# jjjkkyz/NU-NeRF

Measured on AMD Instinct MI355X. Metric: train rays/sec, higher is better.
Workload: dtype f32

## Files before the change

nu_nerf_amd/csrc/gemm.h:

```cpp
#pragma once
#include "nu_common.h"

#include "nu_nerf.h"

int nu_gemm_nt_launch(const NuGemmNT& g, hipStream_t stream);
int nu_gemm_nt_batch_launch(const NuGemmNT* probs, int n, hipStream_t stream);
int nu_gemm_tn_launch(const NuGemmTN& g, hipStream_t stream);
int nu_reduce_push(NuReduceDesc* descs, int* ndesc, int cap, const float* slab, int S, int N1, int N2, int rs,
                   long long ss, float* out, int ldo, float alpha, int accumulate);

int nu_ctx_take(NuOpCtx* c, long long nbytes, int ndesc_needed, hipStream_t stream, float** out, long long* out_bytes);
void nu_ctx_ev_begin(NuOpCtx* c, hipStream_t stream);
void nu_ctx_ev_end(NuOpCtx* c, hipStream_t stream, double kind, double flops, double bytes);
```

nu_nerf_amd/csrc/gemm_epi.h:

```cpp
#pragma once
#include "gemm.h"
#include <type_traits>

#define TBM 128
#define TBN 128
#define TBK 32
#define NT_LDS 36
#define NT_LDSH 40
#define NT_WPC 3

#define EPI_LDS 68

template <int EPI>
static __device__ inline float nu_epi_apply(float v, float bv, float h, float d, float ca, float& out2) {
    out2 = 0.f;
    if (EPI == NU_EPI_BIAS_NONE) return v + bv;
    if (EPI == NU_EPI_BIAS_RELU) return fmaxf(v + bv, 0.0f);
    if (EPI == NU_EPI_BIAS_SOFTPLUS) return nu_softplus100_fast(v + bv);
    if (EPI == NU_EPI_MUL_DRELU) return h > 0.0f ? v : 0.0f;
    if (EPI == NU_EPI_MUL_DSP) return v * (1.0f - nu_exp_m100(h));
    if (EPI == NU_EPI_Q_SP) {
        const float e = nu_exp_m100(h);
        out2 = v * d * 100.0f * e;
        return v * (1.0f - e);
    }
    if (EPI == NU_EPI_B_SP) return v * (1.0f - nu_exp_m100(h)) + ca;
    if (EPI == NU_EPI_B_RELU) return (h > 0.0f ? v : 0.0f) + ca;
    return v;
}

template <int EPI>
struct NtEpiArgs {
    float* C; float* C2; const float* bias; const float* H; const float* D; const float* Cadd;
    unsigned long long* mask;
    int zero_to, act_cols;
    bool vec_ok;
    bool c16, x16;
    static constexpr bool kMaskW = (EPI == NU_EPI_BIAS_RELU);
    static constexpr bool kMaskR = (EPI == NU_EPI_MUL_DRELU || EPI == NU_EPI_B_RELU);
    static constexpr bool kNeedH = (EPI == NU_EPI_MUL_DRELU || EPI == NU_EPI_MUL_DSP || EPI == NU_EPI_Q_SP ||
                                    EPI == NU_EPI_B_SP || EPI == NU_EPI_B_RELU);
    static constexpr bool kNeedD = (EPI == NU_EPI_Q_SP);
    static constexpr bool kNeedAdd = (EPI == NU_EPI_B_SP || EPI == NU_EPI_B_RELU);
    static constexpr bool kBias = (EPI <= NU_EPI_BIAS_SOFTPLUS);
};

template <int EPI, bool H16 = false>
static __device__ inline NtEpiArgs<EPI> nt_epi_args(const NuGemmNT& g, int z) {
    typedef NtEpiArgs<EPI> E;
    E a;
    a.c16 = H16 && (g.bf16 & NU_GEMM_C16) != 0;
    a.x16 = H16 && (g.bf16 & NU_GEMM_X16) != 0;
    const int ec = a.c16 ? 2 : 4, ex = a.x16 ? 2 : 4;
    auto off = [](const float* p, long long elems, int eb) { return reinterpret_cast<const float*>(reinterpret_cast<const char*>(p) + elems * eb); };
    a.C = const_cast<float*>(off(g.C, (long long)z * g.sC, ec));
    a.C2 = g.C2 ? const_cast<float*>(off(g.C2, (long long)z * g.sC2, ec)) : nullptr;
    a.bias = g.bias ? g.bias + (long long)z * g.sBias : nullptr;
    a.H = g.H ? off(g.H, (long long)z * g.sH, ex) : nullptr;
    a.D = g.D ? off(g.D, (long long)z * g.sD, ex) : nullptr;
    a.Cadd = g.Cadd ? off(g.Cadd, (long long)z * g.sCadd, ex) : nullptr;
    a.zero_to = g.zero_to > g.N ? g.zero_to : g.N;
    a.act_cols = g.act_cols > 0 ? g.act_cols : 0x7fffffff;
    a.mask = (E::kMaskW || E::kMaskR) ? g.mask : nullptr;
    const uintptr_t mc = a.c16 ? 7 : 15, mx = a.x16 ? 7 : 15;
    bool v = (((uintptr_t)a.C & mc) == 0) && ((g.ldc & 3) == 0);
    if (E::kNeedH) v = v && (((uintptr_t)a.H & mx) == 0) && ((g.ldh & 3) == 0);
    if (E::kNeedD) v = v && (((uintptr_t)a.D & mx) == 0) && ((g.ldd & 3) == 0) && (((uintptr_t)a.C2 & mc) == 0) && ((g.ldc2 & 3) == 0);
    if (E::kNeedAdd) v = v && (((uintptr_t)a.Cadd & mx) == 0) && ((g.ldadd & 3) == 0);
    a.vec_ok = v;
    return a;
}

static __device__ __forceinline__ f32x4 nu_bf16x4_to_f32(uint2 r) {
    f32x4 o;
    o[0] = __uint_as_float(r.x << 16); o[1] = __uint_as_float(r.x & 0xffff0000u);
// ... 17 lines not shown
    else base[idx] = v;
}

template <int EPI>
static __device__ inline unsigned long long* nt_mask_words(const NtEpiArgs<EPI>& ea, const NuGemmNT& g, int mt, int nt, int z, int ntn, int wid) {
    const int ct = g.mask_ct0 + z * ntn + nt;
    return (ea.mask && ct < g.mask_nct) ? ea.mask + ((((long long)mt * g.mask_nct + ct) * 4 + wid) * 64) : nullptr;
}

template <int EPI, int NBH, bool H16 = false, int TMN = 2>
static __device__ __forceinline__ void nt_epilogue(const NuGemmNT& g, const NtEpiArgs<EPI>& ea, f32x16 (&acc)[TMN][2], float* scr,
                                                   int m0, int n0, unsigned long long* mwave, unsigned mlo, unsigned mhi,
                                                   int lane, int wid, int tm0 = 0) {
    typedef NtEpiArgs<EPI> E;
    constexpr bool kMaskW = E::kMaskW, kMaskR = E::kMaskR, kNeedH = E::kNeedH, kNeedD = E::kNeedD, kNeedAdd = E::kNeedAdd, kBias = E::kBias;
    float* const C = ea.C; float* const C2 = ea.C2;
    const float* const bias = ea.bias; const float* const H = ea.H; const float* const D = ea.D; const float* const Cadd = ea.Cadd;
    const int zero_to = ea.zero_to, act_cols = ea.act_cols;
    const bool vec_ok = ea.vec_ok;
    const bool c16 = H16 && ea.c16, x16 = H16 && ea.x16;
    const int ec = c16 ? 2 : 4, ex = x16 ? 2 : 4;
    const int li = lane & 31, lh = lane >> 5;
    const int wr = wid >> 1, wc = wid & 1;
    unsigned wlo = 0, whi = 0;
    const int colq = (lane & 15) * 4;
    const int gcol = n0 + wc * 64 + colq;
    float bv[4] = {0.f, 0.f, 0.f, 0.f};
    if (kBias && bias) {
#pragma unroll
        for (int e = 0; e < 4; ++e) bv[e] = (gcol + e < g.N) ? bias[gcol + e] : 0.f;
    }
    const bool full = vec_ok && (gcol + 3 < g.N) && (gcol + 3 < act_cols || gcol >= act_cols);
    const int wcol0 = n0 + wc * 64, wrow0 = m0 + wr * 64;
    const bool slab_full = vec_ok && (wrow0 + 64 <= g.M) && (wcol0 + 64 <= g.N) && (wcol0 + 64 <= act_cols || wcol0 >= act_cols);
    const bool slab_plain = kNeedH && wcol0 >= act_cols;
    const int uwid = __builtin_amdgcn_readfirstlane(wid);
    const long long urow0 = m0 + (uwid >> 1) * 64, ucol0 = n0 + (uwid & 1) * 64;
    const unsigned lrow = lane >> 4;
    char* const Cu = reinterpret_cast<char*>(C) + (urow0 * g.ldc + ucol0) * ec;
    char* const C2u = kNeedD ? reinterpret_cast<char*>(C2) + (urow0 * g.ldc2 + ucol0) * ec : nullptr;
    const char* const Hu = kNeedH ? reinterpret_cast<const char*>(H) + (urow0 * g.ldh + ucol0) * ex : nullptr;
    const char* const Du = kNeedD ? reinterpret_cast<const char*>(D) + (urow0 * g.ldd + ucol0) * ex : nullptr;
    const char* const Au = kNeedAdd ? reinterpret_cast<const char*>(Cadd) + (urow0 * g.ldadd + ucol0) * ex : nullptr;
    const unsigned oC = (lrow * (unsigned)g.ldc + (unsigned)colq) * (unsigned)ec, oC2 = (lrow * (unsigned)g.ldc2 + (unsigned)colq) * (unsigned)ec;
    const unsigned oH = (lrow * (unsigned)g.ldh + (unsigned)colq) * (unsigned)ex, oD = (lrow * (unsigned)g.ldd + (unsigned)colq) * (unsigned)ex;
    const unsigned oA = (lrow * (unsigned)g.ldadd + (unsigned)colq) * (unsigned)ex;
#pragma unroll
    for (int tt = 0; tt < TMN; ++tt) {
        const int tm = tm0 + tt;
#pragma unroll
        for (int tn = 0; tn < 2; ++tn)
#pragma unroll
            for (int r = 0; r < 16; ++r)
                scr[((r & 3) + 8 * (r >> 2) + 4 * lh) * EPI_LDS + tn * 32 + li] = acc[tt][tn][r];
        if (slab_full) {
            auto fast = [&](auto ub_c, auto pl_c, auto c16_c, auto x16_c) {
                constexpr bool UB = decltype(ub_c)::value, PL = decltype(pl_c)::value;
                constexpr bool c16 = decltype(c16_c)::value, x16 = decltype(x16_c)::value;
                constexpr int ec = c16 ? 2 : 4, ex = x16 ? 2 : 4;
                constexpr int NB = kNeedH ? NBH : 4;
#pragma unroll
                for (int hb = 0; hb < 8 / NB; ++hb) {
                    f32x4 v4[NB], h4[NB], d4[NB], c4v[NB];
#pragma unroll
                    for (int ii = 0; ii < NB; ++ii) {
                        const int i = hb * NB + ii;
                        const long long roff = (long long)(tm * 32 + i * 4);
                        v4[ii] = *reinterpret_cast<const f32x4*>(&scr[(i * 4 + (lane >> 4)) * EPI_LDS + colq]);
                        if (kNeedH && !PL && !UB) h4[ii] = nt_ld4<H16>(Hu + roff * g.ldh * ex + oH, x16);
                        if (kNeedD && !PL) d4[ii] = nt_ld4<H16>(Du + roff * g.ldd * ex + oD, x16);
                        if (kNeedAdd && !PL) c4v[ii] = nt_ld4<H16>(Au + roff * g.ldadd * ex + oA, x16);
                    }
#pragma unroll
                    for (int ii = 0; ii < NB; ++ii) {
                        const int i = hb * NB + ii;
                        const long long roff = (long long)(tm * 32 + i * 4);
                        f32x4 o4, o24;
#pragma unroll
                        for (int e = 0; e < 4; ++e) {
                            float o2 = 0.f;
                            const float v = g.alpha * v4[ii][e];
                            if constexpr (PL) {
                                o4[e] = v;
                            } else if constexpr (kMaskR && UB) {
                                const int src = (tm * 8 + i) * 4 + e;
                                const unsigned long long w = ((unsigned long long)(unsigned)__builtin_amdgcn_readlane(mhi, src) << 32) |
                                                             (unsigned)__builtin_amdgcn_readlane(mlo, src);
                                float sel;
                                asm("s_nop 1\n\tv_cndmask_b32_e64 %0, 0, %1, %2" : "=v"(sel) : "v"(v), "s"(w));
                                o4[e] = kNeedAdd ? sel + c4v[ii][e] : sel;
                            } else {
                                o4[e] = nu_epi_apply<EPI>(v, bv[e], kNeedH ? h4[ii][e] : 0.f, kNeedD ? d4[ii][e] : 0.f,
                                                          kNeedAdd ? c4v[ii][e] : 0.f, o2);
                            }
                            o24[e] = o2;
                        }
                        nt_st4<H16>(Cu + roff * g.ldc * ec + oC, o4, c16);
                        if (kNeedD) nt_st4<H16>(C2u + roff * g.ldc2 * ec + oC2, o24, c16);
                        if constexpr (kMaskW && UB) {
#pragma unroll
                            for (int e = 0; e < 4; ++e) {
                                const unsigned long long bits = __ballot(o4[e] > 0.f);
                                const bool mine = lane == (tm * 8 + i) * 4 + e;
                                wlo = mine ? (unsigned)bits : wlo;
                                whi = mine ? (unsigned)(bits >> 32) : whi;
                            }
                        }
                    }
// ... 26 lines not shown
                if (row < g.M) {
                if (full) {
                    f32x4 h4 = {0.f, 0.f, 0.f, 0.f}, d4 = h4, c4v = h4, o4, o24;
                    const bool plain = gcol >= act_cols;
                    if (kMaskR && mwave) {
                        if (!plain) {
#pragma unroll
                            for (int e = 0; e < 4; ++e) {
                                const int src = (tm * 8 + i) * 4 + e;
                                const unsigned lo = __builtin_amdgcn_readlane(mlo, src), hi = __builtin_amdgcn_readlane(mhi, src);
                                h4[e] = (((lane < 32 ? lo : hi) >> (lane & 31)) & 1u) ? 1.0f : 0.0f;
                            }
                        }
                    } else if (kNeedH && !plain) h4 = nt_ld4<H16>(reinterpret_cast<const char*>(H) + ((long long)row * g.ldh + gcol) * ex, x16);
                    if (kNeedD && !plain) d4 = nt_ld4<H16>(reinterpret_cast<const char*>(D) + ((long long)row * g.ldd + gcol) * ex, x16);
                    if (kNeedAdd && !plain) c4v = nt_ld4<H16>(reinterpret_cast<const char*>(Cadd) + ((long long)row * g.ldadd + gcol) * ex, x16);
#pragma unroll
                    for (int e = 0; e < 4; ++e) {
                        float o2;
                        const float v = g.alpha * v4[e];
                        o4[e] = (kNeedH && plain) ? v : nu_epi_apply<EPI>(v, bv[e], h4[e], d4[e], c4v[e], o2);
                        o24[e] = (kNeedH && plain) ? 0.f : o2;
                    }
                    nt_st4<H16>(reinterpret_cast<char*>(C) + ((long long)row * g.ldc + gcol) * ec, o4, c16);
                    if (kNeedD) nt_st4<H16>(reinterpret_cast<char*>(C2) + ((long long)row * g.ldc2 + gcol) * ec, o24, c16);
                    if (kMaskW) {
#pragma unroll
                        for (int e = 0; e < 4; ++e) pos[e] = o4[e] > 0.f;
                    }
                } else {
#pragma unroll
                    for (int e = 0; e < 4; ++e) {
                        const int col = gcol + e;
                        if (col >= zero_to) continue;
                        float out = 0.f, out2 = 0.f;
                        if (col < g.N) {
                            const float v = g.alpha * v4[e];
                            if (kNeedH && col >= act_cols) {
                                out = v;
                            } else {
                                const float h = kNeedH ? nt_ld1<H16>(H, (long long)row * g.ldh + col, x16) : 0.f;
                                const float d = kNeedD ? nt_ld1<H16>(D, (long long)row * g.ldd + col, x16) : 0.f;
                                const float ca = kNeedAdd ? nt_ld1<H16>(Cadd, (long long)row * g.ldadd + col, x16) : 0.f;
                                out = nu_epi_apply<EPI>(v, bv[e], h, d, ca, out2);
                            }
                        }
                        nt_st1<H16>(C, (long long)row * g.ldc + col, out, c16);
                        if (kNeedD) nt_st1<H16>(C2, (long long)row * g.ldc2 + col, out2, c16);
                    }
                }
                }
                if (kMaskW && mwave) {
#pragma unroll
                    for (int e = 0; e < 4; ++e) {
                        const unsigned long long bits = __ballot(pos[e]);
                        const bool mine = lane == (tm * 8 + i) * 4 + e;
                        wlo = mine ? (unsigned)bits : wlo;
                        whi = mine ? (unsigned)(bits >> 32) : whi;
// ... 9 lines not shown
```

nu_nerf_amd/csrc/gemm_nt.hip:

```cpp
#include "gemm_epi.h"

template <int EPI, int PREC>
__global__ __launch_bounds__(256, PREC == 2 ? 2 : NT_WPC) void gemm_nt_kernel(NuGemmNT g) {
    static_assert(PREC == 1 || PREC == 2, "gemm_nt_kernel covers the bf16 modes only");
    constexpr bool SPLIT = PREC == 2;
    constexpr int kPlane = TBM * NT_LDSH;
    __shared__ __attribute__((aligned(16))) float smem[SPLIT ? 1 : 2][SPLIT ? 3 * kPlane : TBM * NT_LDS];
    __bf16* const hA = reinterpret_cast<__bf16*>(&smem[0][0]);
    __bf16* const hB = hA + (SPLIT ? 3 : 1) * kPlane;

    const int tid = threadIdx.x;
    const int lane = tid & 63;
    const int wid = tid >> 6;
    const int wr = wid >> 1, wc = wid & 1;
    const int z = blockIdx.z;
    const int ntn = (g.N + TBN - 1) / TBN;
    const int mtiles = (g.M + TBM - 1) / TBM;
    const int nslots = ((mtiles + 7) / 8) * 8 * ntn;

    const float* __restrict__ A = g.A + (long long)z * g.sA;
    const float* __restrict__ B = g.B + (long long)z * g.sB;
    const int c4 = tid & 7;
    const int r0 = tid >> 3;
    const int nk = g.K / TBK;
// ... 318 lines not shown
#undef NT2_PIN
        nt_epilogue<EPI, 4, false, TMN>(g, ea, acc, &smem[(cur ^ 1) * NT2_STAGE] + wid * (32 * EPI_LDS), m0, n0, mwave, mlo, mhi, lane, slab, tm0);
        int mtn = 0, ntnx = 0;
        const int jn = next_valid(j + gridDim.x, pi, mtn, ntnx);
        if (jn >= nslots) break;
        __syncthreads();
        j = jn; mt = mtn; nt = ntnx;
    }
}

template <int EPI, int TMN>
__global__ __launch_bounds__(256, 2) void gemm_nt2_kernel(NuGemmNT g) {
    __shared__ __attribute__((aligned(16))) float smem[2 * NT2_STAGE];
    nt2_run<EPI, TMN, false>(&g, nullptr, 1, smem);
}
template <int EPI, int TMN>
__global__ __launch_bounds__(256, 2) void gemm_nt2b_kernel(NuGemmNTBatch b) {
    __shared__ __attribute__((aligned(16))) float smem[2 * NT2_STAGE];
    nt2_run<EPI, TMN, true>(b.p, b.slot0, b.n, smem);
}

int nu_gemm_nt16_launch(const NuGemmNT& g, int groups, long long nslots, hipStream_t stream);
int nu_gemm_nt6_launch(const NuGemmNT& g, int groups, hipStream_t stream);

static int nt_check(const NuGemmNT& g) {
    if (g.N <= 0 || g.K <= 0 || (g.K % TBK) != 0 || g.lda < g.K || g.ldb < g.K) return NU_ERR_ARG;
    if ((g.lda & 3) || (g.ldb & 3)) return NU_ERR_ARG;
    if (((uintptr_t)g.A & 15) || ((uintptr_t)g.B & 15)) return NU_ERR_ARG;
    const int ntn = nu_cdiv(g.N, TBN);
    const long long nslots = (long long)nu_rup(nu_cdiv(g.M, 64), 8) * ntn;
    if (nslots > 0x7fffffffLL) return NU_ERR_ARG;
    const int groups = g.groups > 0 ? g.groups : 1;
    if (g.mask && (g.epi == NU_EPI_BIAS_RELU || g.epi == NU_EPI_MUL_DRELU || g.epi == NU_EPI_B_RELU)) {
        if ((g.N & 3) || (g.ldc & 3) || ((uintptr_t)g.C & 15) || g.mask_nct <= 0 || g.mask_ct0 < 0) return NU_ERR_ARG;
        if (g.epi == NU_EPI_B_RELU && ((g.ldadd & 3) || ((uintptr_t)g.Cadd & 15))) return NU_ERR_ARG;
        if (g.epi == NU_EPI_BIAS_RELU && ((long long)g.mask_ct0 + (long long)groups * ntn > g.mask_nct || (g.N & 63))) return NU_ERR_ARG;
        if (g.act_cols > 0 && (g.act_cols & 63)) return NU_ERR_ARG;
    }
    const int prec = g.bf16 & 3;
    if (prec == 3) return NU_ERR_ARG;
    if ((g.bf16 & ~3) && !(prec == 1 && (g.bf16 & NU_GEMM_B16)) && !(prec == 2 && (g.bf16 & ~3) == NU_GEMM_PRESPLIT_ALWAYS && g.B6))
        return NU_ERR_ARG;
    return NU_OK;
}

static bool nt_small_tiles(long long t128, long long t64) {
    auto round_eff = [&](long long tiles) { return (double)tiles / (double)(nu_cdivl(tiles, 512) * 512); };
    return t128 < 512 || 0.95 * round_eff(t64) > round_eff(t128);
}

int nu_gemm_nt_launch(const NuGemmNT& g, hipStream_t stream) {
    if (g.M <= 0) return NU_OK;
    const int rc = nt_check(g);
    if (rc != NU_OK) return rc;
    const int ntn = nu_cdiv(g.N, TBN);
    const long long nslots = (long long)nu_rup(nu_cdiv(g.M, TBM), 8) * ntn;
    const int groups = g.groups > 0 ? g.groups : 1;
    const int prec = g.bf16 & 3;
    dim3 block(256);
    if (prec == 1 && (g.bf16 & NU_GEMM_B16)) return nu_gemm_nt16_launch(g, groups, nslots, stream);
    const bool nt6_epi = g.epi != NU_EPI_Q_SP && g.epi != NU_EPI_B_SP && g.epi != NU_EPI_B_RELU;
    if (prec == 2 && g.B6 &&
        ((g.bf16 & NU_GEMM_PRESPLIT_ALWAYS) || (nt6_epi && (long long)nu_cdiv(g.M, TBM) * nu_cdiv(g.N, 256) * groups >= 320)))
        return nu_gemm_nt6_launch(g, groups, stream);
    if (prec == 0) {
        const long long t128 = (long long)nu_cdiv(g.M, TBM) * ntn * groups, t64 = (long long)nu_cdiv(g.M, 64) * ntn * groups;
        const bool small = nt_small_tiles(t128, t64);
        const long long nslots2 = small ? (long long)nu_rup(nu_cdiv(g.M, 64), 8) * ntn : nslots;
        long long per = nu_rup(nu_cdiv(512, groups), 8);
        if (per > nslots2) per = nslots2;
        dim3 grid((unsigned)per, 1, groups);
        switch (g.epi) {
#define NU_CASE2(E) case E: if (small) hipLaunchKernelGGL((gemm_nt2_kernel<E, 1>), grid, block, 0, stream, g); \
                            else hipLaunchKernelGGL((gemm_nt2_kernel<E, 2>), grid, block, 0, stream, g); break;
            NU_CASE2(NU_EPI_BIAS_NONE)
            NU_CASE2(NU_EPI_BIAS_RELU)
            NU_CASE2(NU_EPI_BIAS_SOFTPLUS)
            NU_CASE2(NU_EPI_MUL_DRELU)
            NU_CASE2(NU_EPI_MUL_DSP)
            NU_CASE2(NU_EPI_Q_SP)
            NU_CASE2(NU_EPI_B_SP)
            NU_CASE2(NU_EPI_PLAIN)
            NU_CASE2(NU_EPI_B_RELU)
#undef NU_CASE2
            default: return NU_ERR_ARG;
        }
        return nu_launch_status();
    }
    long long per = nu_rup(nu_cdiv(256 * (prec == 2 ? 2 : NT_WPC), groups), 8);
    if (per > nslots) per = nslots;
    dim3 grid((unsigned)per, 1, groups);
    switch (g.epi) {
#define NU_CASE(E) case E: if (prec == 2) hipLaunchKernelGGL((gemm_nt_kernel<E, 2>), grid, block, 0, stream, g); \
                           else hipLaunchKernelGGL((gemm_nt_kernel<E, 1>), grid, block, 0, stream, g); break;
        NU_CASE(NU_EPI_BIAS_NONE)
        NU_CASE(NU_EPI_BIAS_RELU)
        NU_CASE(NU_EPI_BIAS_SOFTPLUS)
        NU_CASE(NU_EPI_MUL_DRELU)
        NU_CASE(NU_EPI_MUL_DSP)
        NU_CASE(NU_EPI_Q_SP)
        NU_CASE(NU_EPI_B_SP)
        NU_CASE(NU_EPI_PLAIN)
        NU_CASE(NU_EPI_B_RELU)
#undef NU_CASE
        default: return NU_ERR_ARG;
    }
    return nu_launch_status();
}

int nu_gemm_nt_batch_launch(const NuGemmNT* probs, int n, hipStream_t stream) {
    int i = 0;
    while (i < n) {
        NuGemmNTBatch b;
        int nb = 0, last = i;
        long long t128 = 0, t64 = 0;
        const int epi = probs[i].epi;
        const bool epi_ok = epi == NU_EPI_BIAS_NONE || epi == NU_EPI_BIAS_RELU || epi == NU_EPI_MUL_DRELU || epi == NU_EPI_PLAIN;
        for (int k = i; k < n && epi_ok; ++k) {
            const NuGemmNT& g = probs[k];
// ... 58 lines not shown
```

nu_nerf_amd/csrc/mlp.hip:

```cpp
#include "gemm.h"


static __device__ inline int nu_find_desc(const NuPackDesc* __restrict__ d, int nd, int row) {
    int lo = 0, hi = nd - 1;
    while (lo < hi) {
        int mid = (lo + hi + 1) >> 1;
        if (d[mid].row_begin <= row) lo = mid; else hi = mid - 1;
    }
    return lo;
}

__global__ __launch_bounds__(64) void pack_kernel(const NuPackDesc* __restrict__ descs, int nd) {
    const int row = blockIdx.x;
    const int lane = threadIdx.x;
    const NuPackDesc d = descs[nu_find_desc(descs, nd, row)];
    const int n = row - d.row_begin;
    const float* __restrict__ v = d.v + (long long)n * d.K;
    float s = d.scale;
    if (d.g) {
        float ss = 0.f;
        for (int k = lane; k < d.K; k += 64) ss += v[k] * v[k];
        ss = nu_wave_sum(ss);
        s *= d.g[n] / sqrtf(ss);
    }
// ... 213 lines not shown
#pragma clang fp contract(off)
        float g[NO];
#pragma unroll
        for (int j = 0; j < NO; ++j) {
            g[j] = dy[(long long)p * ldy + j];
            bacc[j] += g[j];
        }
#pragma unroll
        for (int t = 0; t < KQ; ++t) {
            f32x4 d = {0.f, 0.f, 0.f, 0.f};
#pragma unroll
            for (int j = 0; j < NO; ++j) {
                d += g[j] * w[j][t];
                acc[j][t] += g[j] * h[t];
            }
            if (relu_mask) {
#pragma unroll
                for (int e = 0; e < 4; ++e) d[e] = h[t][e] > 0.f ? d[e] : 0.f;
            }
            const long long qi = (long long)p * lddh + cb + 4 * ln + 256 * t;
            if (accumulate) d += sk_ld4<H16>(dH, qi);
            sk_st4<H16>(dH, qi, d);
        }
    };
    int p = p0 + wave * RPW + sub;
    for (; p + STEP < p1; p += 2 * STEP) {
        f32x4 ha[KQ], hb[KQ];
#pragma unroll
        for (int t = 0; t < KQ; ++t) {
            ha[t] = sk_ld4<H16>(H, (long long)p * ldh + cb + 4 * ln + 256 * t);
// ... 58 lines not shown
                                         NuReduceDesc* descs, int* ndesc, int cap, hipStream_t stream) {
    return skinny_bwd_launch(dy, ldy, static_cast<const float*>(H), ldh, P, K, Ws, ldw, NO, static_cast<float*>(dH), lddh, relu_mask,
                             accumulate, dWs, lddw, db, workspace, workspace_bytes, descs, ndesc, cap, true, stream);
}
static int skinny_bwd_launch(const float* dy, int ldy, const float* H, int ldh, int P, int K, const float* Ws, int ldw, int NO, float* dH,
                             int lddh, int relu_mask, int accumulate, float* dWs, int lddw, float* db, void* workspace,
                             long long workspace_bytes, NuReduceDesc* descs, int* ndesc, int cap, bool h16, hipStream_t stream) {
    if (P <= 0) return NU_ERR_ARG;
    if (workspace_bytes < nu_skinny_bwd_workspace_bytes(K, NO)) return NU_ERR_WORKSPACE;
    if (*ndesc + 2 > cap) return NU_ERR_WORKSPACE;
    int blocks = nu_cdiv(P, 64);
    blocks = blocks < NU_SKINNY_BLOCKS ? blocks : NU_SKINNY_BLOCKS;
    float* slab = (float*)workspace;
    float* bslab = slab + (long long)NU_SKINNY_BLOCKS * NO * K;
#define NU_ARGS dy, ldy, H, ldh, P, Ws, ldw, dH, lddh, relu_mask, accumulate, slab, bslab, K
    if ((ldh & 3) || (lddh & 3) || (ldw & 3)) return NU_ERR_ARG;
    if (K == 128) {
        switch (NO) {
            case 1: if (h16) hipLaunchKernelGGL((skinny_bwd_kernel<1, 128, true>), dim3(blocks), dim3(256), 0, stream, NU_ARGS); else hipLaunchKernelGGL((skinny_bwd_kernel<1, 128, false>), dim3(blocks), dim3(256), 0, stream, NU_ARGS); break;
            case 3: if (h16) hipLaunchKernelGGL((skinny_bwd_kernel<3, 128, true>), dim3(blocks), dim3(256), 0, stream, NU_ARGS); else hipLaunchKernelGGL((skinny_bwd_kernel<3, 128, false>), dim3(blocks), dim3(256), 0, stream, NU_ARGS); break;
            default: return NU_ERR_ARG;
        }
    } else if (K == 256) {
        switch (NO) {
            case 1: if (h16) hipLaunchKernelGGL((skinny_bwd_kernel<1, 256, true>), dim3(blocks), dim3(256), 0, stream, NU_ARGS); else hipLaunchKernelGGL((skinny_bwd_kernel<1, 256, false>), dim3(blocks), dim3(256), 0, stream, NU_ARGS); break;
            case 3: if (h16) hipLaunchKernelGGL((skinny_bwd_kernel<3, 256, true>), dim3(blocks), dim3(256), 0, stream, NU_ARGS); else hipLaunchKernelGGL((skinny_bwd_kernel<3, 256, false>), dim3(blocks), dim3(256), 0, stream, NU_ARGS); break;
            default: return NU_ERR_ARG;
        }
    } else if (K == 1024) {
        switch (NO) {
            case 6: if (h16) hipLaunchKernelGGL((skinny_bwd_kernel<6, 256, true>), dim3(blocks, 4), dim3(256), 0, stream, NU_ARGS); else hipLaunchKernelGGL((skinny_bwd_kernel<6, 256, false>), dim3(blocks, 4), dim3(256), 0, stream, NU_ARGS); break;
// ... 148 lines not shown
```

nu_nerf_amd/csrc/mlp_ops.hip:

```cpp
#include "gemm.h"

#define CHK(x) do { const int rc_ = (x); if (rc_ != NU_OK) return rc_; } while (0)

extern "C" int nu_skinny_fwd(const float*, int, int, int, const float*, int, const float*, int, float*, int, hipStream_t);
extern "C" int nu_skinny_fwd_h16(const void*, int, int, int, const float*, int, const float*, int, float*, int, hipStream_t);
extern "C" int nu_skinny_bwd_enqueue_h16(const float*, int, const void*, int, int, int, const float*, int, int, void*, int, int, int,
                                         float*, int, float*, void*, long long, NuReduceDesc*, int*, int, hipStream_t);
extern "C" long long nu_skinny_bwd_workspace_bytes(int, int);
extern "C" int nu_skinny_bwd_enqueue(const float*, int, const float*, int, int, int, const float*, int, int, float*, int, int, int,
                                     float*, int, float*, void*, long long, NuReduceDesc*, int*, int, hipStream_t);
extern "C" long long nu_colsum_workspace_bytes(int);
extern "C" int nu_colsum_enqueue(const float*, int, int, int, float*, int, void*, long long, NuReduceDesc*, int*, int, hipStream_t);
extern "C" int nu_rowscale_dsp(const float*, int, int, int, const float*, float*, int, hipStream_t);
extern "C" long long nu_wgrad_workspace_bytes(int, int, int, int);
extern "C" int nu_wgrad_enqueue(const NuGemmTN*, float*, int, long long, float*, long long, void*, long long, NuReduceDesc*, int*, int,
                                hipStream_t);

static inline int rup_i(int a, int b) { return (a + b - 1) / b * b; }

extern "C" int nu_op_ctx_size(void) { return (int)sizeof(NuOpCtx); }

static inline int ctx_take(NuOpCtx* c, long long nbytes, int ndesc_needed, hipStream_t stream, float** out, long long* out_bytes) {
    return nu_ctx_take(c, nbytes, ndesc_needed, stream, out, out_bytes);
}
// ... 24 lines not shown
    if (h16 && (c->prec != 1 || a.B16 == nullptr)) return NU_ERR_ARG;
    g = NuGemmNT{};
    g.A = a.A; g.lda = a.lda; g.B = h16 ? a.B16 : a.B; g.ldb = a.ldb; g.M = a.M; g.N = a.N; g.K = a.K; g.C = a.C; g.ldc = a.ldc; g.C2 = a.C2;
    g.ldc2 = a.ldc2; g.bias = a.bias; g.H = a.H; g.ldh = a.ldh; g.D = a.D; g.ldd = a.ldd; g.Cadd = a.Cadd; g.ldadd = a.ldadd;
    g.zero_to = a.zero_to; g.act_cols = a.act_cols; g.alpha = 1.0f; g.groups = a.groups; g.sA = a.sA; g.sB = a.sB; g.sC = a.sC;
    g.sBias = a.sBias; g.sH = a.sH; g.epi = a.epi; g.bf16 = h16 ? (1 | NU_GEMM_B16 | a.st) : c->prec; g.mask = a.mask;
    g.mask_nct = a.mask ? a.mask_nct : 0;
    if (c->prec == 2 && !h16) g.B6 = a.B16;
    return NU_OK;
}
static void nt_cost(const NuOpCtx* c, const NtArgs& a, double* flops, double* bytes) {
    const bool h16 = c->h16 != 0;
    const double eA = h16 && (a.st & A16) ? 2 : 4, eB = h16 ? 2 : 4, eC = h16 && (a.st & C16) ? 2 : 4, eX = h16 && (a.st & X16) ? 2 : 4;
    const bool mask_r = a.mask && (a.epi == NU_EPI_MUL_DRELU || a.epi == NU_EPI_B_RELU);
    const double K = a.ktrue ? a.ktrue : a.K, M = a.M, N = a.N;
    *bytes += a.groups * (M * K * eA + N * K * eB + M * N * (eC * (1 + (a.C2 ? 1 : 0)) +
                          eX * ((a.H && !mask_r ? 1 : 0) + (a.D ? 1 : 0) + (a.Cadd ? 1 : 0))));
    *flops += 2.0 * M * N * K * a.groups;
}
static int nt(NuOpCtx* c, const NtArgs& a, hipStream_t stream) {
    if (a.M <= 0) return NU_OK;
    NuGemmNT g;
    CHK(nt_fill(c, a, g));
    ev_begin(c, stream);
    const int rc = nu_gemm_nt_launch(g, stream);
    if (c->ev) {
        double flops = 0, bytes = 0;
        nt_cost(c, a, &flops, &bytes);
        ev_end(c, stream, 0.0, flops, bytes);
    }
    return rc;
}
// ... 234 lines not shown
    return nu_skinny_fwd(b->HV, 128, P, 128, net->rgb.Wp, 128, net->rgb.bias, 3, b->rgb, 4, stream);
}

extern "C" int nu_nerfpp_mlp_bwd(NuOpCtx* c, const NuNerfNet* net, const float* pt, int pt_ld, NuNerfBufs* b, const float* dsig,
                                 const float* drgb, hipStream_t stream) {
    const int P = b->P;
    if (P <= 0) return NU_OK;
    const bool want_in = b->dx != nullptr;
    const int ldf = want_in ? 288 : 256;
    CHK(skinny_bwd(c, drgb, 4, b->HV, 128, P, 128, net->rgb.Wp, 128, 3, b->dHV, 128, 1, net->rgb.dWp, 128, c->flat + net->rgb.db_off, stream));
    CHK(wgrad(c, b->dHV, 128, b->V, 288, P, 128, 288, net->view.dWp, 288, c->flat + net->view.db_off, stream));
    NtArgs gF = {b->dHV, 128, net->view.WpT, net->view.ldT, P, ldf, 128, b->dF, ldf, NU_EPI_PLAIN};
    gF.B16 = w16(c, net->view.WpT16, 0);
    CHK(nt(c, gF, stream));
    CHK(wgrad(c, b->dF, ldf, b->H[8], 256, P, 256, 256, net->feat.dWp, 256, c->flat + net->feat.db_off, stream, NU_TN_B0_16));
    CHK(skinny_bwd(c, dsig, 1, b->H[8], 256, P, 256, net->alpha.Wp, 256, 1, b->dH8a, 256, 1, net->alpha.dWp, 256, c->flat + net->alpha.db_off, stream,
                   true));
    NtArgs g8 = {b->dF, ldf, net->feat.WpT, net->feat.ldT, P, 256, 256, b->dA[8], 256, NU_EPI_B_RELU};
    g8.H = b->H[8]; g8.ldh = 256; g8.Cadd = b->dH8a; g8.ldadd = 256; g8.mask = b->mask[8]; g8.mask_nct = 2;
    g8.B16 = w16(c, net->feat.WpT16, 0); g8.st = C16 | X16;
    CHK(nt(c, g8, stream));
    const float* dA = b->dA[8];
    int lda = 256;
    int dA_i = 8;
    const float* dskip = nullptr;
    for (int i = 7; i >= 0; --i) {
        const NuLin& L = net->pts[i];
        const int ldu = i == 0 ? 96 : (i == 5 ? 352 : 256);
        CHK(wgrad(c, dA, lda, b->H[i], ldu, P, 256, L.Kp, L.dWp, L.ldd, c->flat + L.db_off, stream,
                  (nerfdA16(dA_i) ? NU_TN_A0_16 : 0) | (nerfH16(i) ? NU_TN_B0_16 : 0)));
        if (i > 0) {
            const int st = (nerfdA16(dA_i) ? A16 : 0) | (nerfdA16(i) ? C16 : 0) | (nerfH16(i) ? X16 : 0);
            if (i == 5 && want_in) {
                NtArgs g = {dA, lda, L.WpT, L.ldT, P, 340, 256, b->dA[i], 352, NU_EPI_MUL_DRELU};
// ... 97 lines not shown
```

nu_nerf_amd/engine.py:

```python
import ctypes
import os
import math

import numpy as np
import torch

from . import _lib as L

from ._lib import (GemmNT, GemmTN, ReduceDesc, PackDesc, Lin, WgradItem, OpCtx, SdfNet, SdfBufs, NerfNet, NerfBufs, ShadeNet, BakeNet,
                   ShadeBufs, EPI_BIAS_NONE, EPI_BIAS_RELU, EPI_BIAS_SOFTPLUS, EPI_MUL_DRELU, EPI_MUL_DSP, EPI_Q_SP, EPI_B_SP,
                   EPI_PLAIN, EPI_B_RELU, NU_WGRAD_QUEUE_MAX)

c_int, c_p = ctypes.c_int, ctypes.c_void_p


def rup(a, b):
    return (a + b - 1) // b * b


def addr(t, off=0):
    if t is None:
        return 0
    return t.data_ptr() + t.element_size() * off

# ... 409 lines not shown
           ldadd=0, zero_to=0, act_cols=0, alpha=1.0, groups=1, sA=0, sB=0, sC=0, sC2=0, sBias=0, sH=0, sD=0, sCadd=0,
           ktrue=None, ntrue=None, mask=None, B6=0):
        if M <= 0:
            return
        g = GemmNT(A, lda, B, ldb, M, N, K, C, ldc, C2, ldc2, bias, H, ldh, D, ldd, Cadd, ldadd, zero_to, act_cols,
                   alpha, groups, sA, sB, sC, sC2, sBias, sH, sD, sCadd, epi, self.bf16,
                   mask.data_ptr() if mask is not None else 0, mask._nu_nct if mask is not None else 0, 0, B6)
        kt = self._ktime if self.ktime_on else None
        if kt is not None:
            e0, e1 = self._event_pair()
            e0.record()
        self.lib.nu_gemm_nt_ex(ctypes.byref(g), self.stream())
        if kt is not None:
            e1.record()
            reads_h = bool(H) and not (mask is not None and epi in (EPI_MUL_DRELU, EPI_B_RELU))
            nmat = 1 + (1 if C2 else 0) + (1 if reads_h else 0) + (1 if D else 0) + (1 if Cadd else 0)
            abytes = 4.0 * groups * (M * (ktrue or K) + M * (ntrue or N) * nmat + N * (ktrue or K))
            kt['nt'].append((e0, e1, 2.0 * M * (ntrue or N) * (ktrue or K) * groups, abytes))

    def nt_desc(self, A, lda, B, ldb, M, N, K, C, ldc, epi, *, C2=0, ldc2=0, bias=0, H=0, ldh=0, D=0, ldd=0, Cadd=0, ldadd=0, zero_to=0,
                act_cols=0, alpha=1.0, groups=1, sA=0, sB=0, sC=0, sC2=0, sBias=0, sH=0, sD=0, sCadd=0, mask=None):
        return GemmNT(A, lda, B, ldb, M, N, K, C, ldc, C2, ldc2, bias, H, ldh, D, ldd, Cadd, ldadd, zero_to, act_cols,
                      alpha, groups, sA, sB, sC, sC2, sBias, sH, sD, sCadd, epi, self.bf16,
                      mask.data_ptr() if mask is not None else 0, mask._nu_nct if mask is not None else 0, 0, 0)

    def nt_batch(self, descs):
        descs = [g for g in descs if g.M > 0]
        if not descs:
            return
        arr = (GemmNT * len(descs))(*descs)
        kt = self._ktime if self.ktime_on else None
        if kt is not None:
# ... 535 lines not shown
        b['H'] = H
        sig = e(P)
        self.skinny_fwd(addr(H[8]), 256, P, 256, addr(*self.nerf_alpha.Wp), 256, addr(self.nerf_alpha.b), 1, addr(sig), 1)
        self.nt(addr(H[8]), 256, addr(*self.nerf_feat.Wp), 256, P, 256, 256, addr(V), 288, EPI_BIAS_NONE,
                bias=addr(self.nerf_feat.b))
        HV = e(P, 128)
        self.nt(addr(V), 288, addr(*self.nerf_view.Wp), 288, P, 128, 288, addr(HV), 128, EPI_BIAS_RELU,
                bias=addr(self.nerf_view.b))
        rgb = e(P, 4)
        self.skinny_fwd(addr(HV), 128, P, 128, addr(*self.nerf_rgb.Wp), 128, addr(self.nerf_rgb.b), 3, addr(rgb), 4)
        if alpha_rm is not None:
            lib.nu_nerf_act_fwd(addr(sig), 1, addr(rgb), 4, addr(pt), addr(idx), P, addr(alpha_rm), addr(color_rm), S)
        b.update(V=V, HV=HV, sig=sig, rgb=rgb)
        return b

    def nerf_backward(self, b, pt, idx, dalpha_rm, dcolor_rm, flat, dsig=None, drgb=None, dx=None, ddir=None):
        lib, S, P = self.lib, self.stream(), b['P']
        e = self.empty
        H = b['H']
        want_in = dx is not None
        if dsig is None:
            dsig, drgb = e(P), e(P, 4)
            lib.nu_nerf_act_bwd(addr(b['sig']), 1, addr(b['rgb']), 4, addr(pt), addr(idx), P,
                                addr(dalpha_rm), addr(dcolor_rm), addr(dsig), 1, addr(drgb), 4, S)
        if self._use_c():
            cb = b.get('cb')
            if cb is None:
                cb = NerfBufs(P=P, V=addr(b['V']), HV=addr(b['HV']), sig=addr(b['sig']), rgb=addr(b['rgb']))
                for i in range(9):
                    cb.H[i] = addr(H[i])
                    if i > 0:
                        cb.mask[i] = addr(getattr(H[i], '_nu_mask', None))
            ldf = 288 if want_in else 256
            keep = [e(P, 128), e(P, ldf), self.empty_h(P, 256)]
            cb.dHV, cb.dF, cb.dH8a = (addr(t) for t in keep)
            for i in range(1, 9):
                t = e(P, 352 if want_in else 256) if i == 5 else self.empty_h(P, 256)
                keep.append(t)
                cb.dA[i] = addr(t)
            if want_in:
                t = e(P, 96)
                keep.append(t)
                cb.dE4, cb.dx, cb.ddir = addr(t), addr(dx), addr(ddir)
            else:
                cb.dE4 = cb.dx = cb.ddir = 0
            self._ensure_arena()
            self._ctx.flat = addr(flat)
            lib.nu_nerfpp_mlp_bwd(ctypes.byref(self._ctx), ctypes.byref(self._nerf_net), addr(pt),
                                  pt.shape[1], ctypes.byref(cb), addr(dsig), addr(drgb), S)
            return
        with self.wgrad_batch() as wb:
            dHV = wb.keep(e(P, 128))
            self.skinny_bwd(addr(drgb), 4, addr(b['HV']), 128, P, 128, addr(*self.nerf_rgb.Wp), 128, 3, addr(dHV), 128, 1, 0,
                            addr(*self.nerf_rgb.dWp), 128, addr(flat, self.nerf_rgb.db_off))
            self.wgrad(addr(dHV), 128, addr(b['V']), 288, P, 128, 288, addr(*self.nerf_view.dWp), 288,
                       addr(flat, self.nerf_view.db_off))
            ldf = 288 if want_in else 256
            dF = wb.keep(e(P, ldf))
            self.nt(addr(dHV), 128, addr(*self.nerf_view.WpT), self.nerf_view.ldT, P, ldf, 128, addr(dF), ldf, EPI_PLAIN)
            self.wgrad(addr(dF), ldf, addr(H[8]), 256, P, 256, 256, addr(*self.nerf_feat.dWp), 256,
                       addr(flat, self.nerf_feat.db_off))
            dH8a = wb.keep(e(P, 256))
            self.skinny_bwd(addr(dsig), 1, addr(H[8]), 256, P, 256, addr(*self.nerf_alpha.Wp), 256, 1, addr(dH8a), 256, 1, 0,
                            addr(*self.nerf_alpha.dWp), 256, addr(flat, self.nerf_alpha.db_off))
            dA = wb.keep(e(P, 256))
            self.nt(addr(dF), ldf, addr(*self.nerf_feat.WpT), self.nerf_feat.ldT, P, 256, 256, addr(dA), 256, EPI_B_RELU,
                    H=addr(H[8]), ldh=256, Cadd=addr(dH8a), ldadd=256, mask=getattr(H[8], '_nu_mask', None))
            dskip, lda = None, 256
            for i in range(7, -1, -1):
                lay = self.nerf[i]
                ldu = 96 if i == 0 else (352 if i == 5 else 256)
                self.wgrad(addr(dA), lda, addr(H[i]), ldu, P, 256, lay.Kp, addr(*lay.dWp), lay.ldd, addr(flat, lay.db_off))
                if i > 0:
                    if i == 5 and want_in:
                        nxt = wb.keep(e(P, 352))
                        self.nt(addr(dA), lda, addr(*lay.WpT), lay.ldT, P, 340, 256, addr(nxt), 352, EPI_MUL_DRELU,
                                H=addr(H[i]), ldh=ldu, act_cols=256, zero_to=352, mask=getattr(H[i], '_nu_mask', None))
                        dskip = nxt
                        dA, lda = nxt, 352
                    else:
                        nxt = wb.keep(e(P, 256))
                        self.nt(addr(dA), lda, addr(*lay.WpT), lay.ldT, P, 256, 256, addr(nxt), 256, EPI_MUL_DRELU,
# ... 216 lines not shown
```

Before: 98990.

## Fuse rank-1 alpha-head gradient addend into the NT GEMM epilogue

The alpha head's input gradient (dsig times the alpha weight row) used to be written by skinny_bwd as a full P×256 matrix and then read back in the B_RELU GEMM epilogue. That addend is now computed inside the epilogue from the per-row dsig and per-column weight vectors, so skinny_bwd skips writing dH. This saves a P×256 write plus a read and the buffer allocation. In exchange it adds a new kernel instantiation, ds_bpermute row broadcasts, and extra FLOPs in the epilogue, and the path is disabled for bf16 storage.

```diff
diff --git a/nu_nerf_amd/csrc/gemm.h b/nu_nerf_amd/csrc/gemm.h
--- a/nu_nerf_amd/csrc/gemm.h
+++ b/nu_nerf_amd/csrc/gemm.h
@@ -4,6 +4,7 @@
 #include "nu_nerf.h"
 
 int nu_gemm_nt_launch(const NuGemmNT& g, hipStream_t stream);
+static inline bool nu_nt_rank1(const NuGemmNT& g) { return g.epi == NU_EPI_B_RELU && g.D && g.Cadd && g.ldadd == 0; }
 int nu_gemm_nt_batch_launch(const NuGemmNT* probs, int n, hipStream_t stream);
 int nu_gemm_tn_launch(const NuGemmTN& g, hipStream_t stream);
 int nu_reduce_push(NuReduceDesc* descs, int* ndesc, int cap, const float* slab, int S, int N1, int N2, int rs,
diff --git a/nu_nerf_amd/csrc/gemm_epi.h b/nu_nerf_amd/csrc/gemm_epi.h
--- a/nu_nerf_amd/csrc/gemm_epi.h
+++ b/nu_nerf_amd/csrc/gemm_epi.h
@@ -10,6 +10,8 @@
 #define NT_WPC 3
 
 #define EPI_LDS 68
+
+#define NU_EPI_B_RELU_R1 NU_EPI_COUNT
 
 template <int EPI>
 static __device__ inline float nu_epi_apply(float v, float bv, float h, float d, float ca, float& out2) {
@@ -25,24 +27,37 @@
         return v * (1.0f - e);
     }
     if (EPI == NU_EPI_B_SP) return v * (1.0f - nu_exp_m100(h)) + ca;
-    if (EPI == NU_EPI_B_RELU) return (h > 0.0f ? v : 0.0f) + ca;
+    if (EPI == NU_EPI_B_RELU || EPI == NU_EPI_B_RELU_R1) return (h > 0.0f ? v : 0.0f) + ca;
     return v;
+}
+
+static __device__ __forceinline__ float nu_r1_addend(float r, float c) {
+#pragma clang fp contract(off)
+    const float p = r * c;
+    return 0.f + p;
+}
+static __device__ __forceinline__ float nu_r1_sum(float alpha, float acc, float add) {
+#pragma clang fp contract(off)
+    const float v = alpha * acc;
+    return v + add;
 }
 
 template <int EPI>
 struct NtEpiArgs {
     float* C; float* C2; const float* bias; const float* H; const float* D; const float* Cadd;
+    const float* r1_row;
     unsigned long long* mask;
     int zero_to, act_cols;
     bool vec_ok;
     bool c16, x16;
     static constexpr bool kMaskW = (EPI == NU_EPI_BIAS_RELU);
-    static constexpr bool kMaskR = (EPI == NU_EPI_MUL_DRELU || EPI == NU_EPI_B_RELU);
+    static constexpr bool kMaskR = (EPI == NU_EPI_MUL_DRELU || EPI == NU_EPI_B_RELU || EPI == NU_EPI_B_RELU_R1);
     static constexpr bool kNeedH = (EPI == NU_EPI_MUL_DRELU || EPI == NU_EPI_MUL_DSP || EPI == NU_EPI_Q_SP ||
-                                    EPI == NU_EPI_B_SP || EPI == NU_EPI_B_RELU);
+                                    EPI == NU_EPI_B_SP || EPI == NU_EPI_B_RELU || EPI == NU_EPI_B_RELU_R1);
     static constexpr bool kNeedD = (EPI == NU_EPI_Q_SP);
     static constexpr bool kNeedAdd = (EPI == NU_EPI_B_SP || EPI == NU_EPI_B_RELU);
     static constexpr bool kBias = (EPI <= NU_EPI_BIAS_SOFTPLUS);
+    static constexpr bool kR1 = (EPI == NU_EPI_B_RELU_R1);
 };
 
 template <int EPI, bool H16 = false>
@@ -59,6 +74,7 @@
     a.H = g.H ? off(g.H, (long long)z * g.sH, ex) : nullptr;
     a.D = g.D ? off(g.D, (long long)z * g.sD, ex) : nullptr;
     a.Cadd = g.Cadd ? off(g.Cadd, (long long)z * g.sCadd, ex) : nullptr;
+    a.r1_row = E::kR1 ? g.D + (long long)z * g.sD : nullptr;
     a.zero_to = g.zero_to > g.N ? g.zero_to : g.N;
     a.act_cols = g.act_cols > 0 ? g.act_cols : 0x7fffffff;
     a.mask = (E::kMaskW || E::kMaskR) ? g.mask : nullptr;
@@ -106,6 +122,8 @@
                                                    int lane, int wid, int tm0 = 0) {
     typedef NtEpiArgs<EPI> E;
     constexpr bool kMaskW = E::kMaskW, kMaskR = E::kMaskR, kNeedH = E::kNeedH, kNeedD = E::kNeedD, kNeedAdd = E::kNeedAdd, kBias = E::kBias;
+    constexpr bool kR1 = E::kR1;
+    static_assert(!(kR1 && H16), "the rank-1 addend has no bf16-storage form");
     float* const C = ea.C; float* const C2 = ea.C2;
     const float* const bias = ea.bias; const float* const H = ea.H; const float* const D = ea.D; const float* const Cadd = ea.Cadd;
     const int zero_to = ea.zero_to, act_cols = ea.act_cols;
@@ -126,6 +144,13 @@
     const int wcol0 = n0 + wc * 64, wrow0 = m0 + wr * 64;
     const bool slab_full = vec_ok && (wrow0 + 64 <= g.M) && (wcol0 + 64 <= g.N) && (wcol0 + 64 <= act_cols || wcol0 >= act_cols);
     const bool slab_plain = kNeedH && wcol0 >= act_cols;
+    float cv[4] = {0.f, 0.f, 0.f, 0.f};
+    float rowv = 0.f;
+    if (kR1) {
+#pragma unroll
+        for (int e = 0; e < 4; ++e) cv[e] = (gcol + e < g.N) ? Cadd[gcol + e] : 0.f;
+        rowv = (wrow0 + lane < g.M) ? ea.r1_row[wrow0 + lane] : 0.f;
+    }
     const int uwid = __builtin_amdgcn_readfirstlane(wid);
     const long long urow0 = m0 + (uwid >> 1) * 64, ucol0 = n0 + (uwid & 1) * 64;
     const unsigned lrow = lane >> 4;
@@ -148,12 +173,14 @@
         if (slab_full) {
             auto fast = [&](auto ub_c, auto pl_c, auto c16_c, auto x16_c) {
                 constexpr bool UB = decltype(ub_c)::value, PL = decltype(pl_c)::value;
+                constexpr bool R1 = kR1 && !PL;
                 constexpr bool c16 = decltype(c16_c)::value, x16 = decltype(x16_c)::value;
                 constexpr int ec = c16 ? 2 : 4, ex = x16 ? 2 : 4;
                 constexpr int NB = kNeedH ? NBH : 4;
 #pragma unroll
                 for (int hb = 0; hb < 8 / NB; ++hb) {
                     f32x4 v4[NB], h4[NB], d4[NB], c4v[NB];
+                    float rr[NB];
 #pragma unroll
                     for (int ii = 0; ii < NB; ++ii) {
                         const int i = hb * NB + ii;
@@ -161,7 +188,8 @@
                         v4[ii] = *reinterpret_cast<const f32x4*>(&scr[(i * 4 + (lane >> 4)) * EPI_LDS + colq]);
                         if (kNeedH && !PL && !UB) h4[ii] = nt_ld4<H16>(Hu + roff * g.ldh * ex + oH, x16);
                         if (kNeedD && !PL) d4[ii] = nt_ld4<H16>(Du + roff * g.ldd * ex + oD, x16);
-                        if (kNeedAdd && !PL) c4v[ii] = nt_ld4<H16>(Au + roff * g.ldadd * ex + oA, x16);
+                        if (kNeedAdd && !PL && !R1) c4v[ii] = nt_ld4<H16>(Au + roff * g.ldadd * ex + oA, x16);
+                        if (R1) rr[ii] = __int_as_float(__builtin_amdgcn_ds_bpermute((int)(((unsigned)(tm * 32 + i * 4) + lrow) * 4u), __float_as_int(rowv)));
                     }
 #pragma unroll
                     for (int ii = 0; ii < NB; ++ii) {
@@ -178,12 +206,15 @@
                                 const int src = (tm * 8 + i) * 4 + e;
                                 const unsigned long long w = ((unsigned long long)(unsigned)__builtin_amdgcn_readlane(mhi, src) << 32) |
                                                              (unsigned)__builtin_amdgcn_readlane(mlo, src);
-                                float sel;
-                                asm("s_nop 1\n\tv_cndmask_b32_e64 %0, 0, %1, %2" : "=v"(sel) : "v"(v), "s"(w));
-                                o4[e] = kNeedAdd ? sel + c4v[ii][e] : sel;
+                                float sel, t = v;
+                                if constexpr (R1) t = nu_r1_sum(g.alpha, v4[ii][e], nu_r1_addend(rr[ii], cv[e]));
+                                asm("s_nop 1\n\tv_cndmask_b32_e64 %0, 0, %1, %2" : "=v"(sel) : "v"(t), "s"(w));
+                                o4[e] = (kNeedAdd && !R1) ? sel + c4v[ii][e] : sel;
                             } else {
-                                o4[e] = nu_epi_apply<EPI>(v, bv[e], kNeedH ? h4[ii][e] : 0.f, kNeedD ? d4[ii][e] : 0.f,
-                                                          kNeedAdd ? c4v[ii][e] : 0.f, o2);
+                                float ca = 0.f;
+                                if constexpr (R1) ca = h4[ii][e] > 0.0f ? nu_r1_addend(rr[ii], cv[e]) : 0.0f;
+                                else if constexpr (kNeedAdd) ca = c4v[ii][e];
+                                o4[e] = nu_epi_apply<EPI>(v, bv[e], kNeedH ? h4[ii][e] : 0.f, kNeedD ? d4[ii][e] : 0.f, ca, o2);
                             }
                             o24[e] = o2;
                         }
@@ -240,7 +271,13 @@
                         }
                     } else if (kNeedH && !plain) h4 = nt_ld4<H16>(reinterpret_cast<const char*>(H) + ((long long)row * g.ldh + gcol) * ex, x16);
                     if (kNeedD && !plain) d4 = nt_ld4<H16>(reinterpret_cast<const char*>(D) + ((long long)row * g.ldd + gcol) * ex, x16);
-                    if (kNeedAdd && !plain) c4v = nt_ld4<H16>(reinterpret_cast<const char*>(Cadd) + ((long long)row * g.ldadd + gcol) * ex, x16);
+                    if (kR1) {
+                        if (!plain) {
+                            const float rrow = ea.r1_row[row];
+#pragma unroll
+                            for (int e = 0; e < 4; ++e) c4v[e] = h4[e] > 0.0f ? nu_r1_addend(rrow, cv[e]) : 0.0f;
+                        }
+                    } else if (kNeedAdd && !plain) c4v = nt_ld4<H16>(reinterpret_cast<const char*>(Cadd) + ((long long)row * g.ldadd + gcol) * ex, x16);
 #pragma unroll
                     for (int e = 0; e < 4; ++e) {
                         float o2;
@@ -267,7 +304,9 @@
                             } else {
                                 const float h = kNeedH ? nt_ld1<H16>(H, (long long)row * g.ldh + col, x16) : 0.f;
                                 const float d = kNeedD ? nt_ld1<H16>(D, (long long)row * g.ldd + col, x16) : 0.f;
-                                const float ca = kNeedAdd ? nt_ld1<H16>(Cadd, (long long)row * g.ldadd + col, x16) : 0.f;
+                                float ca = 0.f;
+                                if (kR1) ca = h > 0.0f ? nu_r1_addend(ea.r1_row[row], cv[e]) : 0.0f;
+                                else if (kNeedAdd) ca = nt_ld1<H16>(Cadd, (long long)row * g.ldadd + col, x16);
                                 out = nu_epi_apply<EPI>(v, bv[e], h, d, ca, out2);
                             }
                         }
diff --git a/nu_nerf_amd/csrc/gemm_nt.hip b/nu_nerf_amd/csrc/gemm_nt.hip
--- a/nu_nerf_amd/csrc/gemm_nt.hip
+++ b/nu_nerf_amd/csrc/gemm_nt.hip
@@ -356,6 +356,11 @@
     __shared__ __attribute__((aligned(16))) float smem[2 * NT2_STAGE];
     nt2_run<EPI, TMN, false>(&g, nullptr, 1, smem);
 }
+template <int TMN>
+__global__ __launch_bounds__(256, 2) void gemm_nt2r1_kernel(NuGemmNT g) {
+    __shared__ __attribute__((aligned(16))) float smem[2 * NT2_STAGE];
+    nt2_run<NU_EPI_B_RELU_R1, TMN, false>(&g, nullptr, 1, smem);
+}
 template <int EPI, int TMN>
 __global__ __launch_bounds__(256, 2) void gemm_nt2b_kernel(NuGemmNTBatch b) {
     __shared__ __attribute__((aligned(16))) float smem[2 * NT2_STAGE];
@@ -375,12 +380,13 @@
     const int groups = g.groups > 0 ? g.groups : 1;
     if (g.mask && (g.epi == NU_EPI_BIAS_RELU || g.epi == NU_EPI_MUL_DRELU || g.epi == NU_EPI_B_RELU)) {
         if ((g.N & 3) || (g.ldc & 3) || ((uintptr_t)g.C & 15) || g.mask_nct <= 0 || g.mask_ct0 < 0) return NU_ERR_ARG;
-        if (g.epi == NU_EPI_B_RELU && ((g.ldadd & 3) || ((uintptr_t)g.Cadd & 15))) return NU_ERR_ARG;
+        if (g.epi == NU_EPI_B_RELU && !nu_nt_rank1(g) && ((g.ldadd & 3) || ((uintptr_t)g.Cadd & 15))) return NU_ERR_ARG;
         if (g.epi == NU_EPI_BIAS_RELU && ((long long)g.mask_ct0 + (long long)groups * ntn > g.mask_nct || (g.N & 63))) return NU_ERR_ARG;
         if (g.act_cols > 0 && (g.act_cols & 63)) return NU_ERR_ARG;
     }
     const int prec = g.bf16 & 3;
     if (prec == 3) return NU_ERR_ARG;
+    if (nu_nt_rank1(g) && prec == 1) return NU_ERR_ARG;
     if ((g.bf16 & ~3) && !(prec == 1 && (g.bf16 & NU_GEMM_B16)) && !(prec == 2 && (g.bf16 & ~3) == NU_GEMM_PRESPLIT_ALWAYS && g.B6))
         return NU_ERR_ARG;
     return NU_OK;
@@ -402,7 +408,8 @@
     dim3 block(256);
     if (prec == 1 && (g.bf16 & NU_GEMM_B16)) return nu_gemm_nt16_launch(g, groups, nslots, stream);
     const bool nt6_epi = g.epi != NU_EPI_Q_SP && g.epi != NU_EPI_B_SP && g.epi != NU_EPI_B_RELU;
-    if (prec == 2 && g.B6 &&
+    const bool r1 = nu_nt_rank1(g);
+    if (prec == 2 && g.B6 && !r1 &&
         ((g.bf16 & NU_GEMM_PRESPLIT_ALWAYS) || (nt6_epi && (long long)nu_cdiv(g.M, TBM) * nu_cdiv(g.N, 256) * groups >= 320)))
         return nu_gemm_nt6_launch(g, groups, stream);
     if (prec == 0) {
@@ -412,6 +419,11 @@
         long long per = nu_rup(nu_cdiv(512, groups), 8);
         if (per > nslots2) per = nslots2;
         dim3 grid((unsigned)per, 1, groups);
+        if (r1) {
+            if (small) hipLaunchKernelGGL((gemm_nt2r1_kernel<1>), grid, block, 0, stream, g);
+            else hipLaunchKernelGGL((gemm_nt2r1_kernel<2>), grid, block, 0, stream, g);
+            return nu_launch_status();
+        }
         switch (g.epi) {
 #define NU_CASE2(E) case E: if (small) hipLaunchKernelGGL((gemm_nt2_kernel<E, 1>), grid, block, 0, stream, g); \
                             else hipLaunchKernelGGL((gemm_nt2_kernel<E, 2>), grid, block, 0, stream, g); break;
@@ -432,7 +444,7 @@
     long long per = nu_rup(nu_cdiv(256 * (prec == 2 ? 2 : NT_WPC), groups), 8);
     if (per > nslots) per = nslots;
     dim3 grid((unsigned)per, 1, groups);
-    switch (g.epi) {
+    switch (r1 ? NU_EPI_B_RELU_R1 : g.epi) {
 #define NU_CASE(E) case E: if (prec == 2) hipLaunchKernelGGL((gemm_nt_kernel<E, 2>), grid, block, 0, stream, g); \
                            else hipLaunchKernelGGL((gemm_nt_kernel<E, 1>), grid, block, 0, stream, g); break;
         NU_CASE(NU_EPI_BIAS_NONE)
@@ -445,6 +457,7 @@
         NU_CASE(NU_EPI_PLAIN)
         NU_CASE(NU_EPI_B_RELU)
 #undef NU_CASE
+        case NU_EPI_B_RELU_R1: hipLaunchKernelGGL((gemm_nt_kernel<NU_EPI_B_RELU_R1, 2>), grid, block, 0, stream, g); break;
         default: return NU_ERR_ARG;
     }
     return nu_launch_status();
diff --git a/nu_nerf_amd/csrc/mlp.hip b/nu_nerf_amd/csrc/mlp.hip
--- a/nu_nerf_amd/csrc/mlp.hip
+++ b/nu_nerf_amd/csrc/mlp.hip
@@ -251,6 +251,7 @@
                 d += g[j] * w[j][t];
                 acc[j][t] += g[j] * h[t];
             }
+            if (dH == nullptr) continue;
             if (relu_mask) {
 #pragma unroll
                 for (int e = 0; e < 4; ++e) d[e] = h[t][e] > 0.f ? d[e] : 0.f;
@@ -339,7 +340,7 @@
     float* slab = (float*)workspace;
     float* bslab = slab + (long long)NU_SKINNY_BLOCKS * NO * K;
 #define NU_ARGS dy, ldy, H, ldh, P, Ws, ldw, dH, lddh, relu_mask, accumulate, slab, bslab, K
-    if ((ldh & 3) || (lddh & 3) || (ldw & 3)) return NU_ERR_ARG;
+    if ((ldh & 3) || (dH && (lddh & 3)) || (ldw & 3)) return NU_ERR_ARG;
     if (K == 128) {
         switch (NO) {
             case 1: if (h16) hipLaunchKernelGGL((skinny_bwd_kernel<1, 128, true>), dim3(blocks), dim3(256), 0, stream, NU_ARGS); else hipLaunchKernelGGL((skinny_bwd_kernel<1, 128, false>), dim3(blocks), dim3(256), 0, stream, NU_ARGS); break;
diff --git a/nu_nerf_amd/csrc/mlp_ops.hip b/nu_nerf_amd/csrc/mlp_ops.hip
--- a/nu_nerf_amd/csrc/mlp_ops.hip
+++ b/nu_nerf_amd/csrc/mlp_ops.hip
@@ -62,8 +62,9 @@
     const double eA = h16 && (a.st & A16) ? 2 : 4, eB = h16 ? 2 : 4, eC = h16 && (a.st & C16) ? 2 : 4, eX = h16 && (a.st & X16) ? 2 : 4;
     const bool mask_r = a.mask && (a.epi == NU_EPI_MUL_DRELU || a.epi == NU_EPI_B_RELU);
     const double K = a.ktrue ? a.ktrue : a.K, M = a.M, N = a.N;
+    const bool r1 = a.epi == NU_EPI_B_RELU && a.D && a.Cadd && a.ldadd == 0;
     *bytes += a.groups * (M * K * eA + N * K * eB + M * N * (eC * (1 + (a.C2 ? 1 : 0)) +
-                          eX * ((a.H && !mask_r ? 1 : 0) + (a.D ? 1 : 0) + (a.Cadd ? 1 : 0))));
+                          eX * ((a.H && !mask_r ? 1 : 0) + (a.D && !r1 ? 1 : 0) + (a.Cadd && !r1 ? 1 : 0))) + (r1 ? 4.0 * (M + N) : 0.0));
     *flops += 2.0 * M * N * K * a.groups;
 }
 static int nt(NuOpCtx* c, const NtArgs& a, hipStream_t stream) {
@@ -328,10 +329,13 @@
     gF.B16 = w16(c, net->view.WpT16, 0);
     CHK(nt(c, gF, stream));
     CHK(wgrad(c, b->dF, ldf, b->H[8], 256, P, 256, 256, net->feat.dWp, 256, c->flat + net->feat.db_off, stream, NU_TN_B0_16));
-    CHK(skinny_bwd(c, dsig, 1, b->H[8], 256, P, 256, net->alpha.Wp, 256, 1, b->dH8a, 256, 1, net->alpha.dWp, 256, c->flat + net->alpha.db_off, stream,
-                   true));
+    const bool r1 = !c->h16;
+    CHK(skinny_bwd(c, dsig, 1, b->H[8], 256, P, 256, net->alpha.Wp, 256, 1, r1 ? nullptr : b->dH8a, 256, 1, net->alpha.dWp, 256,
+                   c->flat + net->alpha.db_off, stream, true));
     NtArgs g8 = {b->dF, ldf, net->feat.WpT, net->feat.ldT, P, 256, 256, b->dA[8], 256, NU_EPI_B_RELU};
-    g8.H = b->H[8]; g8.ldh = 256; g8.Cadd = b->dH8a; g8.ldadd = 256; g8.mask = b->mask[8]; g8.mask_nct = 2;
+    g8.H = b->H[8]; g8.ldh = 256; g8.mask = b->mask[8]; g8.mask_nct = 2;
+    if (r1) { g8.D = dsig; g8.Cadd = net->alpha.Wp; }
+    else { g8.Cadd = b->dH8a; g8.ldadd = 256; }
     g8.B16 = w16(c, net->feat.WpT16, 0); g8.st = C16 | X16;
     CHK(nt(c, g8, stream));
     const float* dA = b->dA[8];
diff --git a/nu_nerf_amd/engine.py b/nu_nerf_amd/engine.py
--- a/nu_nerf_amd/engine.py
+++ b/nu_nerf_amd/engine.py
@@ -447,8 +447,9 @@
         if kt is not None:
             e1.record()
             reads_h = bool(H) and not (mask is not None and epi in (EPI_MUL_DRELU, EPI_B_RELU))
-            nmat = 1 + (1 if C2 else 0) + (1 if reads_h else 0) + (1 if D else 0) + (1 if Cadd else 0)
-            abytes = 4.0 * groups * (M * (ktrue or K) + M * (ntrue or N) * nmat + N * (ktrue or K))
+            r1 = epi == EPI_B_RELU and bool(D) and bool(Cadd) and ldadd == 0
+            nmat = 1 + (1 if C2 else 0) + (1 if reads_h else 0) + (1 if D and not r1 else 0) + (1 if Cadd and not r1 else 0)
+            abytes = 4.0 * groups * (M * (ktrue or K) + M * (ntrue or N) * nmat + N * (ktrue or K) + ((M + N) if r1 else 0))
             kt['nt'].append((e0, e1, 2.0 * M * (ntrue or N) * (ktrue or K) * groups, abytes))
 
     def nt_desc(self, A, lda, B, ldb, M, N, K, C, ldc, epi, *, C2=0, ldc2=0, bias=0, H=0, ldh=0, D=0, ldd=0, Cadd=0, ldadd=0, zero_to=0,
@@ -1014,7 +1015,7 @@
         b.update(V=V, HV=HV, sig=sig, rgb=rgb)
         return b
 
-    def nerf_backward(self, b, pt, idx, dalpha_rm, dcolor_rm, flat, dsig=None, drgb=None, dx=None, ddir=None):
+    def nerf_backward(self, b, pt, idx, dalpha_rm, dcolor_rm, flat, dsig=None, drgb=None, dx=None, ddir=None, _matrix_addend=False):
         lib, S, P = self.lib, self.stream(), b['P']
         e = self.empty
         H = b['H']
@@ -1032,8 +1033,12 @@
                     if i > 0:
                         cb.mask[i] = addr(getattr(H[i], '_nu_mask', None))
             ldf = 288 if want_in else 256
-            keep = [e(P, 128), e(P, ldf), self.empty_h(P, 256)]
-            cb.dHV, cb.dF, cb.dH8a = (addr(t) for t in keep)
+            keep = [e(P, 128), e(P, ldf)]
+            cb.dHV, cb.dF = (addr(t) for t in keep)
+            cb.dH8a = 0
+            if self.h16:
+                keep.append(self.empty_h(P, 256))
+                cb.dH8a = addr(keep[-1])
             for i in range(1, 9):
                 t = e(P, 352 if want_in else 256) if i == 5 else self.empty_h(P, 256)
                 keep.append(t)
@@ -1060,12 +1065,13 @@
             self.nt(addr(dHV), 128, addr(*self.nerf_view.WpT), self.nerf_view.ldT, P, ldf, 128, addr(dF), ldf, EPI_PLAIN)
             self.wgrad(addr(dF), ldf, addr(H[8]), 256, P, 256, 256, addr(*self.nerf_feat.dWp), 256,
                        addr(flat, self.nerf_feat.db_off))
-            dH8a = wb.keep(e(P, 256))
+            dH8a = wb.keep(e(P, 256)) if _matrix_addend else None
             self.skinny_bwd(addr(dsig), 1, addr(H[8]), 256, P, 256, addr(*self.nerf_alpha.Wp), 256, 1, addr(dH8a), 256, 1, 0,
                             addr(*self.nerf_alpha.dWp), 256, addr(flat, self.nerf_alpha.db_off))
             dA = wb.keep(e(P, 256))
+            add = dict(Cadd=addr(dH8a), ldadd=256) if _matrix_addend else dict(D=addr(dsig), Cadd=addr(*self.nerf_alpha.Wp))
             self.nt(addr(dF), ldf, addr(*self.nerf_feat.WpT), self.nerf_feat.ldT, P, 256, 256, addr(dA), 256, EPI_B_RELU,
-                    H=addr(H[8]), ldh=256, Cadd=addr(dH8a), ldadd=256, mask=getattr(H[8], '_nu_mask', None))
+                    H=addr(H[8]), ldh=256, mask=getattr(H[8], '_nu_mask', None), **add)
             dskip, lda = None, 256
             for i in range(7, -1, -1):
                 lay = self.nerf[i]
```

Result: slower. 97820 (-1.2%).
